# gaspachoo/EEG2Video

Measured on AMD Instinct MI355X. Metric: 6-frame 288x512 clips/sec (50-step DDIM), higher is better.
Workload: dtype f32; 1 GPU; 1xMI355X: batch=8/GPU synthetic latents [B,4,6,36,64] + [B,77,768] cond, 50-step DDIM, CFG 12.5, 288x512x6 VAE decode, fp32 (BASELINE configs[1]); clips_per_gpu=8, ddim_steps=50, unet_samples_per_ddim_step=16, weights=random-init SD-v1-4 architecture, counter RNG seed 42/43, collective=none

## Files before the change

### eeg2video_amd/_lib.py

```python
from __future__ import annotations

import ctypes as C
import os

_HERE = os.path.dirname(os.path.abspath(__file__))
LIB_PATH = os.environ.get("E2V_LIB_PATH") or os.path.join(_HERE, "lib", "libeeg2video_hip.so")

c_int64_p = C.POINTER(C.c_int64)
c_float_p = C.c_void_p


class E2VConfig(C.Structure):
    _fields_ = [
        ("in_channels", C.c_int), ("out_channels", C.c_int),
        ("block_out_channels", C.c_int * 4),
        ("layers_per_block", C.c_int), ("cross_attention_dim", C.c_int), ("attention_heads", C.c_int),
        ("norm_num_groups", C.c_int), ("norm_eps", C.c_float), ("flip_sin_to_cos", C.c_int), ("freq_shift", C.c_float),
        ("vae_in_channels", C.c_int), ("vae_latent_channels", C.c_int),
        ("vae_block_out_channels", C.c_int * 4),
        ("vae_layers_per_block", C.c_int), ("vae_norm_num_groups", C.c_int), ("vae_norm_eps", C.c_float),
        ("vae_scaling_factor", C.c_double),
        ("num_train_timesteps", C.c_int), ("beta_start", C.c_double), ("beta_end", C.c_double),
        ("steps_offset", C.c_int),
        ("sem_in_features", C.c_int), ("sem_hidden", C.c_int), ("sem_tokens", C.c_int),
# ... 27 lines not shown
    "e2v_unet_forward_ft": (_i, [_ctx, _p, C.POINTER(C.c_float), _i, _p, _i, _i, _i, _i, _i, _p, _stream]),
    "e2v_ddim_cfg_step": (_i, [_ctx, _p, _p, _p, _p, _i64, _f, _i64, _i64, _stream]),
    "e2v_vae_decode": (_i, [_ctx, _p, _i, _i, _i, _i, _i, _p, _stream]),
    "e2v_vae_encode": (_i, [_ctx, _p, _i, _i, _i, _p, _p, _stream]),
    "e2v_generate": (_i, [_ctx, _p, _p, _p, _i, _i, _i, _i, _i, _i, _i, _f, _f, _p, _p, _stream]),
    "e2v_semantic_predict": (_i, [_ctx, _p, _i, _p, _stream]),
    "e2v_dana_noise": (_i, [_ctx, _p, _p, _p, c_int64_p, _i, _f, _i, _i, _i, _i, _i, _p, _stream]),
    "e2v_frames_to_uint8": (_i, [_ctx, _p, _p, _i64, _stream]),
    "e2v_cfg_combine": (_i, [_ctx, _p, _p, _f, _p, _i64, _stream]),
    "e2v_lincomb": (_i, [_ctx, _i, C.POINTER(C.c_void_p), C.POINTER(C.c_float), _p, _i64, _stream]),
    "e2v_ddim_next_step": (_i, [_ctx, _p, _p, _p, _i64, _i64, _i, _stream]),
    "e2v_ddim_invert": (_i, [_ctx, _p, _p, _i, _i, _i, _i, _i, _i, _p, _p, _stream]),
    "e2v_set_compute_dtype": (_i, [_ctx, _i]),
    "e2v_set_conv_algo": (_i, [_ctx, _i]),
    "e2v_device_bytes": (_i64, [_ctx]),
    "e2v_comm_unique_id": (_i, [_p]),
    "e2v_comm_init": (_i, [_ctx, _p, _i, _i]),
    "e2v_comm_world": (_i, [_ctx]),
    "e2v_allgather_frames": (_i, [_ctx, _p, _i64, _i, _p, _stream]),
    "e2v_comm_destroy": (_i, [_ctx]),
    "e2v_profile_begin": (_i, [_ctx]),
    "e2v_profile_end": (_i64, [_ctx, C.c_char_p, _i64]),
    "e2v_op_conv3x3": (_i, [_ctx, _p, _i, _p, _i, _i, _i, _i, _i, _i, _i, _i, _i, _i, _p, _p, _i, _p, _i, _p, _p, _stream]),
    "e2v_op_linear": (_i, [_ctx, _p, _i, _i64, _i, _p, _p, _i, _p, _i, _p, _stream]),
    "e2v_op_groupnorm": (_i, [_ctx, _p, _i, _p, _i, _i, _i, _i, _f, _p, _p, _i, _p, _stream]),
    "e2v_op_layernorm": (_i, [_ctx, _p, _i64, _i, _p, _p, _f, _p, _stream]),
    "e2v_op_attention": (_i, [_ctx, _p, _i, _p, _p, _i, _p, _i, _i, _i, _i, _i, _i, _i, _i, _f, _stream]),
    "e2v_op_temporal_attention": (_i, [_ctx, _p, _p, _i, _i, _i, _i, _i, _f, _stream]),
    "e2v_op_to_channels_last": (_i, [_ctx, _p, _p, _i, _i, _i, _i, _stream]),
    "e2v_op_from_channels_last": (_i, [_ctx, _p, _i, _p, _i, _i, _i, _stream]),
    "e2v_op_set_knob": (_i, [C.c_char_p, _i]),
    "e2v_op_rowblock_sums": (_i, [_ctx, _p, _i64, _i, _p, _stream]),
    "e2v_op_describe_dispatch": (_i, [_ctx, _i, _i, _i, _i, _i, _i, C.c_char_p, _i64, c_int64_p]),
    "e2v_op_unet_forward_taps": (_i, [_ctx, _p, c_int64_p, _i, _p, _i, _i, _i, _i, _i, _p, _p, _i64, c_int64_p, C.POINTER(_i), _stream]),
}

_lib = None


def load() -> C.CDLL:
    global _lib
    if _lib is not None:
        return _lib
    if not os.path.isfile(LIB_PATH):
        raise ImportError(
            f"{LIB_PATH} not found: the HIP extension has not been built. "
# ... 16 lines not shown
```

### eeg2video_amd/csrc/api.cpp

```cpp
#include <cmath>
#include <cstdlib>
#include <cstring>
#include <unordered_map>
#include <mutex>

#include "../../include/eeg2video_hip_ops.h"
#include "h16.h"
#include "model.h"
#include "prof.h"

using namespace e2v;

namespace {

std::string g_create_error;

template <typename Fn>
e2v_status guarded(e2v_ctx* ctx, Fn&& fn) {
    try {
        if (ctx && !dry_run()) {
            E2V_REQUIRE(ctx->device >= 0, E2V_ESTATE, "host-only context (device = -1): no GPU work possible");
            E2V_HIP(hipSetDevice(ctx->device));
        }
        fn();
// ... 645 lines not shown
            }
        } else if (const int wm = c->conv_wino_tile(cin, cout, stride, pad_lo, Hi, Wi, Ho, Wo)) {
            Act u(c->pool, (int64_t)(wm + 2) * (wm + 2) * cout, cin);
            wino_pack_weights(w_oihw, u.p, cout, cin, wm, s);
            Act u3;
            if (c->x3_compute) {
                const size_t n = (size_t)(wm + 2) * (wm + 2) * cout * cin;
                u3 = Act(c->pool, (int64_t)((3 * n + 1) / 2 + 1023) / 1024, 1024);
                split_bf16x3(u.p, u3.p, n, n, s);
            }
            conv3_wino(c, d, wm, u.p, u3.p, nullptr, 0, s);
        } else {
            const int ld32 = conv3x3_packed_ld(cin, 32);
            Act wp(c->pool, cout, ld32);
            pack_conv3x3(w_oihw, wp.p, cout, cin, 32, s);
            IgemmArgs g = conv3_igemm(d);
            g.w = wp.p; g.ldw = ld32;
            igemm(g, s);
        }
        E2V_HIP(hipGetLastError());
    });
}

e2v_status e2v_op_linear(e2v_ctx* c, const float* x, int ldx, int64_t M, int K, const float* w, const float* bias, int N,
                         const float* resid, int geglu, float* out, e2v_stream stream) {
    if (!c) return E2V_EINVAL;
    return guarded(c, [&] {
        E2V_REQUIRE(x && w && out && (c->bf16_compute || (K % 4 == 0 && ldx % 4 == 0)), E2V_EINVAL, "bad linear arguments");
        hipStream_t s = S(c, stream);
        IgemmArgs g;
        g.a0 = x; g.c0 = K; g.lda0 = ldx; g.ldw = K; g.out = out; g.M = (int)M; g.taps = 1; g.resid = resid;
        Act wp, bp;
        if (geglu) {
            E2V_REQUIRE(N % 32 == 0 && bias, E2V_EINVAL, "GEGLU width must be a multiple of 32 and have a bias");
            wp = Act(c->pool, 2 * N, K);
            bp = Act(c->pool, 1, 2 * N);
            geglu_interleave(w, bias, N, K, wp.p, bp.p, s);
            g.w = wp.p; g.bias = bp.p; g.N = 2 * N; g.ldc = N; g.geglu = 1;
        } else {
            g.w = w; g.bias = bias; g.N = N; g.ldc = N; g.ldr = N;
        }
        Act w16, wpad, a16;
        if (c->bf16_compute) {
            const int K8 = (K + 7) / 8 * 8;
            a16 = Act(c->pool, M, K8, true);
            cvt_rows(x, ldx, 0, a16.p, K8, c->h16_mode, M, K, K8, s);
// ... 149 lines not shown
```

### eeg2video_amd/csrc/wino.hip

```cpp
#include "kernels.h"
#include "prof.h"

#include <string>

namespace e2v {

typedef float f32x4 __attribute__((ext_vector_type(4)));

__device__ __forceinline__ float wino_silu(float v) {
    return v * __builtin_amdgcn_rcpf(1.0f + __builtin_amdgcn_exp2f(v * -1.44269504088896340736f));
}

__global__ __launch_bounds__(256) void wino_in_kernel(const WinoArgs p, int img_lo, int nimg, float* __restrict__ V) {
    const int Ctot = p.c0 + p.c1;
    const int CQ = Ctot / 4;
    const int th = (p.Ho + 1) / 2, tw = (p.Wo + 1) / 2;
    const size_t T = (size_t)nimg * th * tw;
    const size_t total = T * CQ;
    const size_t plane = T * Ctot;
    for (size_t i = blockIdx.x * (size_t)blockDim.x + threadIdx.x; i < total; i += (size_t)gridDim.x * blockDim.x) {
        const size_t t = i / CQ;
        const int c = (int)(i - t * CQ) * 4;
        const int img = (int)(t / (th * tw));
        const int rem = (int)(t - (size_t)img * th * tw);
        const int ty = rem / tw, tx = rem - ty * tw;
        const bool second = c >= p.c0;
        const float* __restrict__ src = second ? p.x1 + (c - p.c0) : p.x0 + c;
        const int ld = second ? p.ld1 : p.ld0;
        const size_t img_row = (size_t)(img_lo + img) * p.Hs * p.Ws;
        f32x4 ga = {1.f, 0.f, 1.f, 0.f}, gb = {1.f, 0.f, 1.f, 0.f};
        if (p.gn_scsh) {
            const size_t slab = img_row / (size_t)p.gn_P;
            const float* sc = p.gn_scsh + (slab * Ctot + c) * 2;
            ga = *reinterpret_cast<const f32x4*>(sc);
            gb = *reinterpret_cast<const f32x4*>(sc + 4);
        }
        f32x4 d[4][4];
#pragma unroll
        for (int r = 0; r < 4; ++r) {
            const int iy = 2 * ty - 1 + r;
            const bool yok = (unsigned)iy < (unsigned)p.Ho;
            int sy = yok ? iy : 0;
            if (p.upsample) sy = min((int)floorf((float)sy * p.ups_h), p.Hs - 1);
#pragma unroll
            for (int q = 0; q < 4; ++q) {
                const int ix = 2 * tx - 1 + q;
                const bool ok = yok && (unsigned)ix < (unsigned)p.Wo;
                int sx = ok ? ix : 0;
                if (p.upsample) sx = min((int)floorf((float)sx * p.ups_w), p.Ws - 1);
                f32x4 v = {0.f, 0.f, 0.f, 0.f};
                if (ok) {
                    v = *reinterpret_cast<const f32x4*>(src + (img_row + (size_t)sy * p.Ws + sx) * ld);
                    if (p.gn_scsh) {
                        v[0] = v[0] * ga[0] + ga[1];
                        v[1] = v[1] * ga[2] + ga[3];
                        v[2] = v[2] * gb[0] + gb[1];
                        v[3] = v[3] * gb[2] + gb[3];
                        if (p.gn_silu) {
#pragma unroll
                            for (int e = 0; e < 4; ++e) v[e] = wino_silu(v[e]);
                        }
                    }
                }
                d[r][q] = v;
            }
        }
        f32x4 u[4][4];
#pragma unroll
        for (int q = 0; q < 4; ++q) {
            u[0][q] = d[0][q] - d[2][q];
            u[1][q] = d[1][q] + d[2][q];
            u[2][q] = d[2][q] - d[1][q];
            u[3][q] = d[1][q] - d[3][q];
        }
        float* __restrict__ o = V + t * Ctot + c;
#pragma unroll
        for (int r = 0; r < 4; ++r) {
            *reinterpret_cast<f32x4*>(o + (size_t)(4 * r + 0) * plane) = u[r][0] - u[r][2];
            *reinterpret_cast<f32x4*>(o + (size_t)(4 * r + 1) * plane) = u[r][1] + u[r][2];
            *reinterpret_cast<f32x4*>(o + (size_t)(4 * r + 2) * plane) = u[r][2] - u[r][1];
            *reinterpret_cast<f32x4*>(o + (size_t)(4 * r + 3) * plane) = u[r][1] - u[r][3];
        }
    }
}

__global__ __launch_bounds__(256) void wino_out_kernel(const WinoArgs p, int img_lo, int nimg, const float* __restrict__ Mb) {
    const int NQ = p.N / 4;
    const int th = (p.Ho + 1) / 2, tw = (p.Wo + 1) / 2;
    const size_t T = (size_t)nimg * th * tw;
    const size_t total = T * NQ;
    const size_t plane = T * p.N;
    for (size_t i = blockIdx.x * (size_t)blockDim.x + threadIdx.x; i < total; i += (size_t)gridDim.x * blockDim.x) {
        const size_t t = i / NQ;
        const int n = (int)(i - t * NQ) * 4;
        const int img = (int)(t / (th * tw));
        const int rem = (int)(t - (size_t)img * th * tw);
        const int ty = rem / tw, tx = rem - ty * tw;
        const float* __restrict__ m = Mb + t * p.N + n;
        f32x4 w[2][4];
#pragma unroll
        for (int q = 0; q < 4; ++q) {
            const f32x4 m0 = *reinterpret_cast<const f32x4*>(m + (size_t)(0 + q) * plane);
            const f32x4 m1 = *reinterpret_cast<const f32x4*>(m + (size_t)(4 + q) * plane);
            const f32x4 m2 = *reinterpret_cast<const f32x4*>(m + (size_t)(8 + q) * plane);
            const f32x4 m3 = *reinterpret_cast<const f32x4*>(m + (size_t)(12 + q) * plane);
            w[0][q] = m0 + m1 + m2;
            w[1][q] = m1 - m2 - m3;
        }
        f32x4 bias = {0.f, 0.f, 0.f, 0.f};
        if (p.bias) bias = *reinterpret_cast<const f32x4*>(p.bias + n);
#pragma unroll
        for (int a = 0; a < 2; ++a) {
            const int oy = 2 * ty + a;
            if (oy >= p.Ho) continue;
#pragma unroll
            for (int b = 0; b < 2; ++b) {
                const int ox = 2 * tx + b;
                if (ox >= p.Wo) continue;
                f32x4 y = b == 0 ? w[a][0] + w[a][1] + w[a][2] : w[a][1] - w[a][2] - w[a][3];
                const size_t row = ((size_t)(img_lo + img) * p.Ho + oy) * p.Wo + ox;
                y += bias;
                if (p.rowbias) y += *reinterpret_cast<const f32x4*>(p.rowbias + (row / p.rows_per_sample) * p.rb_ld + n);
                if (p.resid) y += *reinterpret_cast<const f32x4*>(p.resid + row * p.ldr + n);
                *reinterpret_cast<f32x4*>(p.out + row * p.ldc + n) = y;
            }
        }
    }
}

__device__ __forceinline__ void bt6(const f32x4 (&d)[6], f32x4 (&o)[6]) {
    o[0] = 4.f * d[0] - 5.f * d[2] + d[4];
    o[1] = -4.f * (d[1] + d[2]) + d[3] + d[4];
    o[2] = 4.f * (d[1] - d[2]) - d[3] + d[4];
    o[3] = 2.f * (d[3] - d[1]) - d[2] + d[4];
    o[4] = 2.f * (d[1] - d[3]) - d[2] + d[4];
    o[5] = 4.f * d[1] - 5.f * d[3] + d[5];
}
__device__ __forceinline__ void at6(const f32x4 (&m)[6], f32x4 (&o)[4]) {
    const f32x4 a = m[1] + m[2], b = m[1] - m[2], c = m[3] + m[4], e = m[3] - m[4];
    o[0] = m[0] + a + c;
    o[1] = b + 2.f * e;
    o[2] = a + 4.f * c;
    o[3] = b + 8.f * e + m[5];
}

__global__ __launch_bounds__(256) void wino4_in_kernel(const WinoArgs p, int img_lo, int nimg, float* __restrict__ V) {
    const int Ctot = p.c0 + p.c1;
    const int CQ = Ctot / 4;
    const int th = (p.Ho + 3) / 4, tw = (p.Wo + 3) / 4;
    const size_t T = (size_t)nimg * th * tw;
    const size_t total = T * CQ;
    const size_t plane = T * Ctot;
    for (size_t i = blockIdx.x * (size_t)blockDim.x + threadIdx.x; i < total; i += (size_t)gridDim.x * blockDim.x) {
        const size_t t = i / CQ;
        const int c = (int)(i - t * CQ) * 4;
        const int img = (int)(t / (th * tw));
        const int rem = (int)(t - (size_t)img * th * tw);
        const int ty = rem / tw, tx = rem - ty * tw;
        const bool second = c >= p.c0;
        const float* __restrict__ src = second ? p.x1 + (c - p.c0) : p.x0 + c;
        const int ld = second ? p.ld1 : p.ld0;
        const size_t img_row = (size_t)(img_lo + img) * p.Hs * p.Ws;
        f32x4 ga = {1.f, 0.f, 1.f, 0.f}, gb = {1.f, 0.f, 1.f, 0.f};
        if (p.gn_scsh) {
            const size_t slab = img_row / (size_t)p.gn_P;
            const float* sc = p.gn_scsh + (slab * Ctot + c) * 2;
            ga = *reinterpret_cast<const f32x4*>(sc);
            gb = *reinterpret_cast<const f32x4*>(sc + 4);
        }
        f32x4 u[6][6];
#pragma unroll
        for (int q = 0; q < 6; ++q) {
            const int ix = 4 * tx - 1 + q;
            const bool xok = (unsigned)ix < (unsigned)p.Wo;
            int sx = xok ? ix : 0;
            if (p.upsample) sx = min((int)floorf((float)sx * p.ups_w), p.Ws - 1);
            f32x4 d[6];
#pragma unroll
            for (int r = 0; r < 6; ++r) {
                const int iy = 4 * ty - 1 + r;
                const bool ok = xok && (unsigned)iy < (unsigned)p.Ho;
                int sy = ok ? iy : 0;
                if (p.upsample) sy = min((int)floorf((float)sy * p.ups_h), p.Hs - 1);
                f32x4 v = {0.f, 0.f, 0.f, 0.f};
                if (ok) {
                    v = *reinterpret_cast<const f32x4*>(src + (img_row + (size_t)sy * p.Ws + sx) * ld);
                    if (p.gn_scsh) {
                        v[0] = v[0] * ga[0] + ga[1];
                        v[1] = v[1] * ga[2] + ga[3];
                        v[2] = v[2] * gb[0] + gb[1];
                        v[3] = v[3] * gb[2] + gb[3];
                        if (p.gn_silu) {
#pragma unroll
                            for (int e = 0; e < 4; ++e) v[e] = wino_silu(v[e]);
                        }
                    }
                }
                d[r] = v;
            }
            f32x4 o[6];
            bt6(d, o);
#pragma unroll
            for (int r = 0; r < 6; ++r) u[r][q] = o[r];
        }
        float* __restrict__ o = V + t * Ctot + c;
#pragma unroll
        for (int r = 0; r < 6; ++r) {
            f32x4 v[6];
            bt6(u[r], v);
#pragma unroll
            for (int q = 0; q < 6; ++q) *reinterpret_cast<f32x4*>(o + (size_t)(6 * r + q) * plane) = v[q];
        }
    }
}

__global__ __launch_bounds__(256) void wino4_out_kernel(const WinoArgs p, int img_lo, int nimg, const float* __restrict__ Mb) {
    const int NQ = p.N / 4;
    const int th = (p.Ho + 3) / 4, tw = (p.Wo + 3) / 4;
    const size_t T = (size_t)nimg * th * tw;
    const size_t total = T * NQ;
    const size_t plane = T * p.N;
    for (size_t i = blockIdx.x * (size_t)blockDim.x + threadIdx.x; i < total; i += (size_t)gridDim.x * blockDim.x) {
        const size_t t = i / NQ;
        const int n = (int)(i - t * NQ) * 4;
        const int img = (int)(t / (th * tw));
        const int rem = (int)(t - (size_t)img * th * tw);
        const int ty = rem / tw, tx = rem - ty * tw;
        const float* __restrict__ m = Mb + t * p.N + n;
        f32x4 w[4][6];
#pragma unroll
        for (int q = 0; q < 6; ++q) {
            f32x4 col[6];
#pragma unroll
            for (int r = 0; r < 6; ++r) col[r] = *reinterpret_cast<const f32x4*>(m + (size_t)(6 * r + q) * plane);
            f32x4 o[4];
            at6(col, o);
#pragma unroll
            for (int a = 0; a < 4; ++a) w[a][q] = o[a];
        }
        f32x4 bias = {0.f, 0.f, 0.f, 0.f};
        if (p.bias) bias = *reinterpret_cast<const f32x4*>(p.bias + n);
#pragma unroll
        for (int a = 0; a < 4; ++a) {
            const int oy = 4 * ty + a;
            if (oy >= p.Ho) continue;
            f32x4 y[4];
            at6(w[a], y);
#pragma unroll
            for (int b = 0; b < 4; ++b) {
                const int ox = 4 * tx + b;
                if (ox >= p.Wo) continue;
                const size_t row = ((size_t)(img_lo + img) * p.Ho + oy) * p.Wo + ox;
                f32x4 v = y[b] + bias;
                if (p.rowbias) v += *reinterpret_cast<const f32x4*>(p.rowbias + (row / p.rows_per_sample) * p.rb_ld + n);
                if (p.resid) v += *reinterpret_cast<const f32x4*>(p.resid + row * p.ldr + n);
                *reinterpret_cast<f32x4*>(p.out + row * p.ldc + n) = v;
            }
        }
    }
}

__global__ void wino4_weight_kernel(const float* __restrict__ w, float* __restrict__ U, int cout, int cin) {
    const size_t total = (size_t)cout * cin;
    const float G[6][3] = {{0.25f, 0.f, 0.f}, {-1.f / 6, -1.f / 6, -1.f / 6}, {-1.f / 6, 1.f / 6, -1.f / 6},
                           {1.f / 24, 1.f / 12, 1.f / 6}, {1.f / 24, -1.f / 12, 1.f / 6}, {0.f, 0.f, 1.f}};
    for (size_t i = blockIdx.x * (size_t)blockDim.x + threadIdx.x; i < total; i += (size_t)gridDim.x * blockDim.x) {
        const float* g = w + i * 9;
        float t[6][3];
#pragma unroll
        for (int r = 0; r < 6; ++r)
#pragma unroll
            for (int x = 0; x < 3; ++x) t[r][x] = G[r][0] * g[x] + G[r][1] * g[3 + x] + G[r][2] * g[6 + x];
#pragma unroll
        for (int r = 0; r < 6; ++r)
#pragma unroll
            for (int q = 0; q < 6; ++q)
                U[(size_t)(6 * r + q) * total + i] = t[r][0] * G[q][0] + t[r][1] * G[q][1] + t[r][2] * G[q][2];
    }
}

__global__ void wino_weight_kernel(const float* __restrict__ w, float* __restrict__ U, int cout, int cin) {
// ... 20 lines not shown

void wino_pack_weights(const float* w_oihw, float* U, int cout, int cin, int m, hipStream_t s) {
    const size_t total = (size_t)cout * cin;
    const int blocks = (int)((total + 255) / 256 < 4096 ? (total + 255) / 256 : 4096);
    if (m == 4) E2V_KLAUNCH(wino4_weight_kernel, dim3(blocks), dim3(256), 0, s, w_oihw, U, cout, cin);
    else E2V_KLAUNCH(wino_weight_kernel, dim3(blocks), dim3(256), 0, s, w_oihw, U, cout, cin);
}

static inline size_t wino_tiles(const WinoArgs& a, int nimg) {
    return (size_t)nimg * ((a.Ho + a.m - 1) / a.m) * ((a.Wo + a.m - 1) / a.m);
}

size_t wino_workspace_floats(const WinoArgs& a, int nimg) {
    return (size_t)(a.m + 2) * (a.m + 2) * wino_tiles(a, nimg) * (size_t)(a.c0 + a.c1 + a.N);
}

int wino_chunk_images(const WinoArgs& a, size_t max_floats) {
    const size_t per_img = wino_workspace_floats(a, 1);
    size_t n = max_floats / (per_img ? per_img : 1);
    if (n < 1) n = 1;
    return (int)(n < (size_t)a.nimg ? n : (size_t)a.nimg);
}

void wino_conv3x3(const WinoArgs& a, float* ws, int chunk_images, hipStream_t s) {
    const int Ctot = a.c0 + a.c1;
    const int P = (a.m + 2) * (a.m + 2);
    for (int lo = 0; lo < a.nimg; lo += chunk_images) {
        const int n = a.nimg - lo < chunk_images ? a.nimg - lo : chunk_images;
        const size_t T = wino_tiles(a, n);
        float* V = ws;
        float* Mb = ws + (size_t)P * T * Ctot;
        {
            const size_t total = T * (Ctot / 4);
            const double px = (double)a.m * a.m;
            std::string nm = a.gn_scsh ? "wino_in_gn_silu" : "wino_in";
            if (prof_detail())
                nm += " T" + std::to_string(T) + " C" + std::to_string(Ctot) + " m" + std::to_string(a.m) + (a.c1 ? " cat" : "") + (a.upsample ? " up" : "");
            ProfScope ps(nm.c_str(), 2.0 * P * T * Ctot, 4.0 * ((px + P) * T * Ctot), s);
            const int blocks = (int)((total + 255) / 256 < 65536 ? (total + 255) / 256 : 65536);
            if (a.m == 4) E2V_KLAUNCH(wino4_in_kernel, dim3(blocks), dim3(256), 0, s, a, lo, n, V);
            else E2V_KLAUNCH(wino_in_kernel, dim3(blocks), dim3(256), 0, s, a, lo, n, V);
        }
        IgemmArgs g;
        g.a0 = V; g.c0 = Ctot; g.lda0 = Ctot; g.w = a.U; g.ldw = Ctot; g.ldw16 = Ctot;
        g.out = Mb; g.ldc = a.N; g.M = (int)T; g.N = a.N; g.taps = 1;
        g.batch = P; g.sa0 = (long long)T * Ctot; g.sw = (long long)a.N * Ctot; g.sout = (long long)T * a.N;
        if (a.U3) { g.x3 = 1; g.w3 = a.U3; g.w3_plane = (long long)P * a.N * Ctot; }
        igemm(g, s);
        {
            const size_t total = T * (a.N / 4);
            const double px = (double)a.m * a.m;
            std::string nm = "wino_out";
            if (prof_detail())
                nm += " T" + std::to_string(T) + " N" + std::to_string(a.N) + " m" + std::to_string(a.m) + (a.resid ? " res" : "") + (a.rowbias ? " temb" : "");
            ProfScope ps(nm.c_str(), 1.5 * P * T * a.N, 4.0 * (P * T * a.N + px * T * a.N * (a.resid ? 2 : 1)), s);
            const int blocks = (int)((total + 255) / 256 < 65536 ? (total + 255) / 256 : 65536);
            if (a.m == 4) E2V_KLAUNCH(wino4_out_kernel, dim3(blocks), dim3(256), 0, s, a, lo, n, Mb);
            else E2V_KLAUNCH(wino_out_kernel, dim3(blocks), dim3(256), 0, s, a, lo, n, Mb);
        }
    }
}

}
```

### eeg2video_amd/engine.py

```python
from __future__ import annotations

import ctypes as C
from typing import Dict, Iterable, Mapping, Optional, Sequence, Tuple

import numpy as np
import torch

from . import _lib
from .weights import SemanticConfig, UNetConfig, VAEConfig

_ERRORS = {
    _lib.E2V_EINVAL: ValueError,
    _lib.E2V_ESHAPE: ValueError,
    _lib.E2V_ENOWEIGHT: RuntimeError,
    _lib.E2V_EHIP: RuntimeError,
    _lib.E2V_ESTATE: RuntimeError,
}


def _stream() -> int:
    return torch.cuda.current_stream().cuda_stream


class Engine:
# ... 336 lines not shown

    def allgather_frames(self, frames: torch.Tensor, as_uint8: bool = False) -> torch.Tensor:
        world = self.lib.e2v_comm_world(self.ctx)
        if world <= 0:
            raise RuntimeError("allgather_frames: no communicator (Engine.comm_init first)")
        v = self._dev(frames, "frames")
        out = torch.empty((world * v.shape[0],) + tuple(v.shape[1:]), device=self.device, dtype=torch.uint8 if as_uint8 else torch.float32)
        self._check(self.lib.e2v_allgather_frames(self.ctx, v.data_ptr(), v.numel(), int(as_uint8), out.data_ptr(), _stream()))
        return out

    def op_conv3x3(self, x0, w, bias=None, x1=None, *, n_img, Hs, Ws, Hi=None, Wi=None, stride=1, pad_lo=1, pad_hi=1,
                   rowbias=None, rows_per_sample=1, resid=None):
        Hi, Wi = Hi or Hs, Wi or Ws
        Ho = (Hi + pad_lo + pad_hi - 3) // stride + 1
        Wo = (Wi + pad_lo + pad_hi - 3) // stride + 1
        cout = w.shape[0]
        out = torch.empty((n_img * Ho * Wo, cout), device=self.device, dtype=torch.float32)
        p = lambda t: t.data_ptr() if t is not None else None
        self._check(self.lib.e2v_op_conv3x3(self.ctx, x0.data_ptr(), x0.shape[1], p(x1), x1.shape[1] if x1 is not None else 0,
                                            n_img, Hs, Ws, Hi, Wi, Ho, Wo, stride, pad_lo, w.data_ptr(), p(bias), cout,
                                            p(rowbias), rows_per_sample, p(resid), out.data_ptr(), _stream()))
        return out

    def op_linear(self, x, w, bias=None, resid=None, geglu=False):
        m, k = x.shape
        n = w.shape[0] // 2 if geglu else w.shape[0]
        out = torch.empty((m, n), device=self.device, dtype=torch.float32)
        p = lambda t: t.data_ptr() if t is not None else None
        self._check(self.lib.e2v_op_linear(self.ctx, x.data_ptr(), x.stride(0), m, k, w.data_ptr(), p(bias), n, p(resid),
                                           int(geglu), out.data_ptr(), _stream()))
        return out

    def op_rowblock_sums(self, x):
        rows, c = x.shape
        out = torch.empty((rows // 64, c, 2), device=self.device, dtype=torch.float32)
        self._check(self.lib.e2v_op_rowblock_sums(self.ctx, x.data_ptr(), rows, c, out.data_ptr(), _stream()))
        return out

    def op_groupnorm(self, x0, gamma, beta, *, samples, P, groups, eps, silu=False, x1=None):
        c = x0.shape[1] + (x1.shape[1] if x1 is not None else 0)
        out = torch.empty((samples * P, c), device=self.device, dtype=torch.float32)
        self._check(self.lib.e2v_op_groupnorm(self.ctx, x0.data_ptr(), x0.shape[1], x1.data_ptr() if x1 is not None else None,
                                              x1.shape[1] if x1 is not None else 0, samples, P, groups, float(eps),
                                              gamma.data_ptr(), beta.data_ptr(), int(silu), out.data_ptr(), _stream()))
        return out

# ... 55 lines not shown
```

### include/eeg2video_hip_ops.h

```cpp
#ifndef EEG2VIDEO_HIP_OPS_H
#define EEG2VIDEO_HIP_OPS_H

#include "eeg2video_hip.h"

#ifdef __cplusplus
extern "C" {
#endif

e2v_status e2v_op_conv3x3(e2v_ctx* ctx, const float* x0, int c0, const float* x1, int c1, int n_img, int Hs, int Ws,
                          int Hi, int Wi, int Ho, int Wo, int stride, int pad_lo, const float* w_oihw, const float* bias,
                          int cout, const float* rowbias, int rows_per_sample, const float* resid, float* out,
                          e2v_stream stream);

e2v_status e2v_op_linear(e2v_ctx* ctx, const float* x, int ldx, int64_t M, int K, const float* w, const float* bias,
                         int N, const float* resid, int geglu, float* out, e2v_stream stream);

e2v_status e2v_op_groupnorm(e2v_ctx* ctx, const float* x0, int c0, const float* x1, int c1, int samples, int P,
                            int groups, float eps, const float* gamma, const float* beta, int silu, float* out,
                            e2v_stream stream);

e2v_status e2v_op_layernorm(e2v_ctx* ctx, const float* x, int64_t rows, int C, const float* gamma, const float* beta,
                            float eps, float* out, e2v_stream stream);

e2v_status e2v_op_attention(e2v_ctx* ctx, const float* q, int ldq, const float* k, const float* v, int ldkv, float* o,
                            int ldo, int n, int F, int heads, int D, int Nq, int Nk, int mode, float scale,
                            e2v_stream stream);

e2v_status e2v_op_temporal_attention(e2v_ctx* ctx, const float* qkv, float* out, int n, int F, int HW, int heads, int D,
                                     float scale, e2v_stream stream);

e2v_status e2v_op_to_channels_last(e2v_ctx* ctx, const float* in, float* out, int n, int C, int Cpad, int FHW,
                                   e2v_stream stream);
e2v_status e2v_op_from_channels_last(e2v_ctx* ctx, const float* in, int ld, float* out, int n, int C, int FHW,
                                     e2v_stream stream);

// ... 15 lines not shown
```

Measured before the change: 0.5895 clips/s.

## Specialize Winograd transform kernels by template and use 32-bit plane offsets

The Winograd input and output transform kernels become templates on GroupNorm fusion, rowbias form and residual presence, so those runtime branches drop out. All global loads are issued ahead of the arithmetic (with scheduling barriers), addresses use 32-bit per-plane offsets with a fast 32-bit divide, and out-of-range taps are masked rather than skipped. A new op entry point fuses GroupNorm+SiLU into the Winograd conv for testing. The change adds register pressure and asserts that offsets fit in 32 bits.

```diff
diff --git a/eeg2video_amd/_lib.py b/eeg2video_amd/_lib.py
--- a/eeg2video_amd/_lib.py
+++ b/eeg2video_amd/_lib.py
@@ -73,6 +73,7 @@
     "e2v_profile_begin": (_i, [_ctx]),
     "e2v_profile_end": (_i64, [_ctx, C.c_char_p, _i64]),
     "e2v_op_conv3x3": (_i, [_ctx, _p, _i, _p, _i, _i, _i, _i, _i, _i, _i, _i, _i, _i, _p, _p, _i, _p, _i, _p, _p, _stream]),
+    "e2v_op_conv3x3_gn": (_i, [_ctx, _p, _i, _p, _i, _i, _i, _i, _i, _i, _i, _i, _i, _i, _i, _i, _f, _p, _p, _p, _p, _i, _p, _i, _p, _p, _stream]),
     "e2v_op_linear": (_i, [_ctx, _p, _i, _i64, _i, _p, _p, _i, _p, _i, _p, _stream]),
     "e2v_op_groupnorm": (_i, [_ctx, _p, _i, _p, _i, _i, _i, _i, _f, _p, _p, _i, _p, _stream]),
     "e2v_op_layernorm": (_i, [_ctx, _p, _i64, _i, _p, _p, _f, _p, _stream]),
diff --git a/eeg2video_amd/csrc/api.cpp b/eeg2video_amd/csrc/api.cpp
--- a/eeg2video_amd/csrc/api.cpp
+++ b/eeg2video_amd/csrc/api.cpp
@@ -691,6 +691,51 @@
     });
 }
 
+e2v_status e2v_op_conv3x3_gn(e2v_ctx* c, const float* x0, int c0, const float* x1, int c1, int n_img, int Hs, int Ws, int Hi, int Wi,
+                             int Ho, int Wo, int stride, int pad_lo, int gn_P, int groups, float eps, const float* gamma,
+                             const float* beta, const float* w_oihw, const float* bias, int cout, const float* rowbias,
+                             int rows_per_sample, const float* resid, float* out, e2v_stream stream) {
+    if (!c) return E2V_EINVAL;
+    const int cin = c0 + c1;
+    const int64_t rows = (int64_t)n_img * Hs * Ws;
+    if (!(x0 && gamma && beta && w_oihw && out && c0 > 0 && c0 % 4 == 0 && c1 >= 0 && c1 % 4 == 0 && (c1 == 0 || x1) && cout > 0 && n_img > 0 &&
+          Hs > 0 && Ws > 0 && groups > 0 && cin % groups == 0 && gn_P > 0 && rows % gn_P == 0)) {
+        c->err = "bad conv3x3_gn arguments";
+        return E2V_EINVAL;
+    }
+    const int wm = c->conv_wino_tile(cin, cout, stride, pad_lo, Hi, Wi, Ho, Wo);
+    if (wm == 0) {
+        c->err = "conv: fused GroupNorm needs the Winograd path";
+        return E2V_ESHAPE;
+    }
+    return guarded(c, [&] {
+        hipStream_t s = S(c, stream);
+        const int samples = (int)(rows / gn_P);
+        Act part(c->pool, (int64_t)samples * groupnorm_chunks(gn_P), cin * 2);
+        Act sc(c->pool, samples, cin * 2);
+        GroupNormArgs a;
+        a.x0 = x0; a.x1 = x1; a.c0 = c0; a.c1 = c1; a.ld0 = c0; a.ld1 = c1; a.gamma = gamma; a.beta = beta;
+        a.samples = samples; a.P = gn_P; a.groups = groups; a.eps = eps;
+        a.ws_part = part.p; a.ws_scale = sc.p;
+        groupnorm_stats(a, s);
+        Conv3 d;
+        d.x0 = x0; d.c0 = c0; d.x1 = x1; d.c1 = c1; d.nimg = n_img; d.Hs = Hs; d.Ws = Ws;
+        d.Hi = Hi; d.Wi = Wi; d.Ho = Ho; d.Wo = Wo; d.stride = stride; d.pad = pad_lo;
+        d.cout = cout; d.out = out; d.bias = bias;
+        d.rowbias = rowbias; d.rb_ld = cout; d.rows_per_sample = rows_per_sample > 0 ? rows_per_sample : 1; d.resid = resid;
+        Act u(c->pool, (int64_t)(wm + 2) * (wm + 2) * cout, cin);
+        wino_pack_weights(w_oihw, u.p, cout, cin, wm, s);
+        Act u3;
+        if (c->x3_compute) {
+            const size_t n = (size_t)(wm + 2) * (wm + 2) * cout * cin;
+            u3 = Act(c->pool, (int64_t)((3 * n + 1) / 2 + 1023) / 1024, 1024);
+            split_bf16x3(u.p, u3.p, n, n, s);
+        }
+        conv3_wino(c, d, wm, u.p, u3.p, sc.p, gn_P, s);
+        E2V_HIP(hipGetLastError());
+    });
+}
+
 e2v_status e2v_op_linear(e2v_ctx* c, const float* x, int ldx, int64_t M, int K, const float* w, const float* bias, int N,
                          const float* resid, int geglu, float* out, e2v_stream stream) {
     if (!c) return E2V_EINVAL;
diff --git a/eeg2video_amd/csrc/wino.hip b/eeg2video_amd/csrc/wino.hip
--- a/eeg2video_amd/csrc/wino.hip
+++ b/eeg2video_amd/csrc/wino.hip
@@ -1,16 +1,61 @@
 #include "kernels.h"
 #include "prof.h"
-
+#include "runtime.h"
+
+#include <algorithm>
 #include <string>
 
 namespace e2v {
 
 typedef float f32x4 __attribute__((ext_vector_type(4)));
+typedef unsigned u32x4 __attribute__((ext_vector_type(4)));
 
 __device__ __forceinline__ float wino_silu(float v) {
     return v * __builtin_amdgcn_rcpf(1.0f + __builtin_amdgcn_exp2f(v * -1.44269504088896340736f));
 }
 
+__device__ __forceinline__ size_t wino_div(size_t a, size_t b) {
+    return ((a | b) >> 32) == 0 ? (size_t)((unsigned)a / (unsigned)b) : a / b;
+}
+
+#define WINO_GLOBAL __attribute__((address_space(1)))
+__device__ __forceinline__ f32x4 wino_plane_load(const float* plane_base, unsigned byte_off) {
+    asm("" : "+s"(plane_base));
+    return *reinterpret_cast<const WINO_GLOBAL f32x4*>((const WINO_GLOBAL char*)plane_base + byte_off);
+}
+__device__ __forceinline__ void wino_plane_store(float* plane_base, unsigned byte_off, f32x4 v) {
+    asm("" : "+s"(plane_base));
+    *reinterpret_cast<WINO_GLOBAL f32x4*>((WINO_GLOBAL char*)plane_base + byte_off) = v;
+}
+
+template <bool GN>
+__device__ __forceinline__ f32x4 wino_act(f32x4 v, const f32x4& ga, const f32x4& gb, bool ok) {
+    if (GN) {
+        v[0] = v[0] * ga[0] + ga[1];
+        v[1] = v[1] * ga[2] + ga[3];
+        v[2] = v[2] * gb[0] + gb[1];
+        v[3] = v[3] * gb[2] + gb[3];
+#pragma unroll
+        for (int e = 0; e < 4; ++e) v[e] = wino_silu(v[e]);
+    }
+    const u32x4 keep = ok ? ~0u : 0u;
+    return __builtin_bit_cast(f32x4, __builtin_bit_cast(u32x4, v) & keep);
+}
+
+template <int PATCH>
+__device__ __forceinline__ void wino_patch_offsets(int o0, int n_out, int n_src, bool upsample, float ups, unsigned step,
+                                                   unsigned (&off)[PATCH], bool (&ok)[PATCH]) {
+#pragma unroll
+    for (int r = 0; r < PATCH; ++r) {
+        const int i = o0 - 1 + r;
+        ok[r] = (unsigned)i < (unsigned)n_out;
+        int s = ok[r] ? i : 0;
+        if (upsample) s = min((int)floorf((float)s * ups), n_src - 1);
+        off[r] = (unsigned)s * step;
+    }
+}
+
+template <bool GN>
 __global__ __launch_bounds__(256) void wino_in_kernel(const WinoArgs p, int img_lo, int nimg, float* __restrict__ V) {
     const int Ctot = p.c0 + p.c1;
     const int CQ = Ctot / 4;
@@ -19,52 +64,36 @@
     const size_t total = T * CQ;
     const size_t plane = T * Ctot;
     for (size_t i = blockIdx.x * (size_t)blockDim.x + threadIdx.x; i < total; i += (size_t)gridDim.x * blockDim.x) {
-        const size_t t = i / CQ;
+        const size_t t = wino_div(i, CQ);
         const int c = (int)(i - t * CQ) * 4;
-        const int img = (int)(t / (th * tw));
+        const int img = (int)wino_div(t, th * tw);
         const int rem = (int)(t - (size_t)img * th * tw);
         const int ty = rem / tw, tx = rem - ty * tw;
         const bool second = c >= p.c0;
-        const float* __restrict__ src = second ? p.x1 + (c - p.c0) : p.x0 + c;
         const int ld = second ? p.ld1 : p.ld0;
         const size_t img_row = (size_t)(img_lo + img) * p.Hs * p.Ws;
+        const float* __restrict__ src = (second ? p.x1 + (c - p.c0) : p.x0 + c) + img_row * ld;
         f32x4 ga = {1.f, 0.f, 1.f, 0.f}, gb = {1.f, 0.f, 1.f, 0.f};
-        if (p.gn_scsh) {
-            const size_t slab = img_row / (size_t)p.gn_P;
+        if (GN) {
+            const size_t slab = wino_div(img_row, (size_t)p.gn_P);
             const float* sc = p.gn_scsh + (slab * Ctot + c) * 2;
             ga = *reinterpret_cast<const f32x4*>(sc);
             gb = *reinterpret_cast<const f32x4*>(sc + 4);
         }
+        unsigned yo[4], xo[4];
+        bool yok[4], xok[4];
+        wino_patch_offsets<4>(2 * ty, p.Ho, p.Hs, p.upsample, p.ups_h, (unsigned)p.Ws * ld, yo, yok);
+        wino_patch_offsets<4>(2 * tx, p.Wo, p.Ws, p.upsample, p.ups_w, (unsigned)ld, xo, xok);
         f32x4 d[4][4];
 #pragma unroll
-        for (int r = 0; r < 4; ++r) {
-            const int iy = 2 * ty - 1 + r;
-            const bool yok = (unsigned)iy < (unsigned)p.Ho;
-            int sy = yok ? iy : 0;
-            if (p.upsample) sy = min((int)floorf((float)sy * p.ups_h), p.Hs - 1);
-#pragma unroll
-            for (int q = 0; q < 4; ++q) {
-                const int ix = 2 * tx - 1 + q;
-                const bool ok = yok && (unsigned)ix < (unsigned)p.Wo;
-                int sx = ok ? ix : 0;
-                if (p.upsample) sx = min((int)floorf((float)sx * p.ups_w), p.Ws - 1);
-                f32x4 v = {0.f, 0.f, 0.f, 0.f};
-                if (ok) {
-                    v = *reinterpret_cast<const f32x4*>(src + (img_row + (size_t)sy * p.Ws + sx) * ld);
-                    if (p.gn_scsh) {
-                        v[0] = v[0] * ga[0] + ga[1];
-                        v[1] = v[1] * ga[2] + ga[3];
-                        v[2] = v[2] * gb[0] + gb[1];
-                        v[3] = v[3] * gb[2] + gb[3];
-                        if (p.gn_silu) {
-#pragma unroll
-                            for (int e = 0; e < 4; ++e) v[e] = wino_silu(v[e]);
-                        }
-                    }
-                }
-                d[r][q] = v;
-            }
-        }
+        for (int r = 0; r < 4; ++r)
+#pragma unroll
+            for (int q = 0; q < 4; ++q) d[r][q] = *reinterpret_cast<const f32x4*>(src + (yo[r] + xo[q]));
+        __builtin_amdgcn_sched_barrier(0);
+#pragma unroll
+        for (int r = 0; r < 4; ++r)
+#pragma unroll
+            for (int q = 0; q < 4; ++q) d[r][q] = wino_act<GN>(d[r][q], ga, gb, yok[r] && xok[q]);
         f32x4 u[4][4];
 #pragma unroll
         for (int q = 0; q < 4; ++q) {
@@ -73,17 +102,77 @@
             u[2][q] = d[2][q] - d[1][q];
             u[3][q] = d[1][q] - d[3][q];
         }
-        float* __restrict__ o = V + t * Ctot + c;
+        const unsigned vo = ((unsigned)t * Ctot + c) * 4u;
 #pragma unroll
         for (int r = 0; r < 4; ++r) {
-            *reinterpret_cast<f32x4*>(o + (size_t)(4 * r + 0) * plane) = u[r][0] - u[r][2];
-            *reinterpret_cast<f32x4*>(o + (size_t)(4 * r + 1) * plane) = u[r][1] + u[r][2];
-            *reinterpret_cast<f32x4*>(o + (size_t)(4 * r + 2) * plane) = u[r][2] - u[r][1];
-            *reinterpret_cast<f32x4*>(o + (size_t)(4 * r + 3) * plane) = u[r][1] - u[r][3];
-        }
-    }
-}
-
+            wino_plane_store(V + (size_t)(4 * r + 0) * plane, vo, u[r][0] - u[r][2]);
+            wino_plane_store(V + (size_t)(4 * r + 1) * plane, vo, u[r][1] + u[r][2]);
+            wino_plane_store(V + (size_t)(4 * r + 2) * plane, vo, u[r][2] - u[r][1]);
+            wino_plane_store(V + (size_t)(4 * r + 3) * plane, vo, u[r][1] - u[r][3]);
+        }
+    }
+}
+
+template <int M, int RB, bool RES>
+struct WinoTileOut {
+    float* out;
+    const float* res;
+    size_t row0;
+    unsigned yc[M], xc[M], yr[M], xr[M];
+    bool yok[M], xok[M];
+    f32x4 bias, rb;
+    f32x4 r[M][M];
+
+    __device__ __forceinline__ WinoTileOut(const WinoArgs& p, int img, int ty, int tx, int n) {
+        const int oy0 = M * ty, ox0 = M * tx;
+        row0 = ((size_t)img * p.Ho + oy0) * p.Wo + ox0;
+        out = p.out + row0 * p.ldc + n;
+        res = RES ? p.resid + row0 * p.ldr + n : nullptr;
+#pragma unroll
+        for (int a = 0; a < M; ++a) {
+            yok[a] = oy0 + a < p.Ho;
+            xok[a] = ox0 + a < p.Wo;
+            yc[a] = (unsigned)(a * p.Wo) * p.ldc;
+            xc[a] = (unsigned)a * p.ldc;
+            yr[a] = yok[a] ? (unsigned)(a * p.Wo) * p.ldr : 0u;
+            xr[a] = xok[a] ? (unsigned)a * p.ldr : 0u;
+        }
+        bias = f32x4{0.f, 0.f, 0.f, 0.f};
+        rb = bias;
+        if (p.bias) bias = *reinterpret_cast<const f32x4*>(p.bias + n);
+        if (RB == 1) rb = *reinterpret_cast<const f32x4*>(p.rowbias + wino_div(row0, (size_t)p.rows_per_sample) * p.rb_ld + n);
+    }
+    __device__ __forceinline__ void load_resid() {
+        if (!RES) return;
+#pragma unroll
+        for (int a = 0; a < M; ++a)
+#pragma unroll
+            for (int b = 0; b < M; ++b) r[a][b] = *reinterpret_cast<const f32x4*>(res + (yr[a] + xr[b]));
+    }
+    __device__ __forceinline__ void finish(const WinoArgs& p, int n, f32x4 (&y)[M][M]) const {
+#pragma unroll
+        for (int a = 0; a < M; ++a)
+#pragma unroll
+            for (int b = 0; b < M; ++b) asm volatile("" : "+v"(y[a][b]));
+        __builtin_amdgcn_s_waitcnt(0x0F70);
+#pragma unroll
+        for (int a = 0; a < M; ++a)
+#pragma unroll
+            for (int b = 0; b < M; ++b) {
+                if (!(yok[a] && xok[b])) continue;
+                f32x4 v = y[a][b] + bias;
+                if (RB == 1) v += rb;
+                if (RB == 2) {
+                    const size_t row = row0 + (size_t)a * p.Wo + b;
+                    v += *reinterpret_cast<const f32x4*>(p.rowbias + wino_div(row, (size_t)p.rows_per_sample) * p.rb_ld + n);
+                }
+                if (RES) v += r[a][b];
+                *reinterpret_cast<f32x4*>(out + (yc[a] + xc[b])) = v;
+            }
+    }
+};
+
+template <int RB, bool RES>
 __global__ __launch_bounds__(256) void wino_out_kernel(const WinoArgs p, int img_lo, int nimg, const float* __restrict__ Mb) {
     const int NQ = p.N / 4;
     const int th = (p.Ho + 1) / 2, tw = (p.Wo + 1) / 2;
@@ -91,40 +180,31 @@
     const size_t total = T * NQ;
     const size_t plane = T * p.N;
     for (size_t i = blockIdx.x * (size_t)blockDim.x + threadIdx.x; i < total; i += (size_t)gridDim.x * blockDim.x) {
-        const size_t t = i / NQ;
+        const size_t t = wino_div(i, NQ);
         const int n = (int)(i - t * NQ) * 4;
-        const int img = (int)(t / (th * tw));
+        const int img = (int)wino_div(t, th * tw);
         const int rem = (int)(t - (size_t)img * th * tw);
         const int ty = rem / tw, tx = rem - ty * tw;
-        const float* __restrict__ m = Mb + t * p.N + n;
+        const unsigned mo = ((unsigned)t * p.N + n) * 4u;
+        f32x4 mm[16];
+#pragma unroll
+        for (int k = 0; k < 16; ++k) mm[k] = wino_plane_load(Mb + (size_t)k * plane, mo);
+        WinoTileOut<2, RB, RES> tile(p, img_lo + img, ty, tx, n);
+        tile.load_resid();
+        __builtin_amdgcn_sched_barrier(0);
         f32x4 w[2][4];
 #pragma unroll
         for (int q = 0; q < 4; ++q) {
-            const f32x4 m0 = *reinterpret_cast<const f32x4*>(m + (size_t)(0 + q) * plane);
-            const f32x4 m1 = *reinterpret_cast<const f32x4*>(m + (size_t)(4 + q) * plane);
-            const f32x4 m2 = *reinterpret_cast<const f32x4*>(m + (size_t)(8 + q) * plane);
-            const f32x4 m3 = *reinterpret_cast<const f32x4*>(m + (size_t)(12 + q) * plane);
-            w[0][q] = m0 + m1 + m2;
-            w[1][q] = m1 - m2 - m3;
-        }
-        f32x4 bias = {0.f, 0.f, 0.f, 0.f};
-        if (p.bias) bias = *reinterpret_cast<const f32x4*>(p.bias + n);
+            w[0][q] = mm[q] + mm[4 + q] + mm[8 + q];
+            w[1][q] = mm[4 + q] - mm[8 + q] - mm[12 + q];
+        }
+        f32x4 y[2][2];
 #pragma unroll
         for (int a = 0; a < 2; ++a) {
-            const int oy = 2 * ty + a;
-            if (oy >= p.Ho) continue;
-#pragma unroll
-            for (int b = 0; b < 2; ++b) {
-                const int ox = 2 * tx + b;
-                if (ox >= p.Wo) continue;
-                f32x4 y = b == 0 ? w[a][0] + w[a][1] + w[a][2] : w[a][1] - w[a][2] - w[a][3];
-                const size_t row = ((size_t)(img_lo + img) * p.Ho + oy) * p.Wo + ox;
-                y += bias;
-                if (p.rowbias) y += *reinterpret_cast<const f32x4*>(p.rowbias + (row / p.rows_per_sample) * p.rb_ld + n);
-                if (p.resid) y += *reinterpret_cast<const f32x4*>(p.resid + row * p.ldr + n);
-                *reinterpret_cast<f32x4*>(p.out + row * p.ldc + n) = y;
-            }
-        }
+            y[a][0] = w[a][0] + w[a][1] + w[a][2];
+            y[a][1] = w[a][1] - w[a][2] - w[a][3];
+        }
+        tile.finish(p, n, y);
     }
 }
 
@@ -144,6 +224,7 @@
     o[3] = b + 8.f * e + m[5];
 }
 
+template <bool GN>
 __global__ __launch_bounds__(256) void wino4_in_kernel(const WinoArgs p, int img_lo, int nimg, float* __restrict__ V) {
     const int Ctot = p.c0 + p.c1;
     const int CQ = Ctot / 4;
@@ -152,68 +233,54 @@
     const size_t total = T * CQ;
     const size_t plane = T * Ctot;
     for (size_t i = blockIdx.x * (size_t)blockDim.x + threadIdx.x; i < total; i += (size_t)gridDim.x * blockDim.x) {
-        const size_t t = i / CQ;
+        const size_t t = wino_div(i, CQ);
         const int c = (int)(i - t * CQ) * 4;
-        const int img = (int)(t / (th * tw));
+        const int img = (int)wino_div(t, th * tw);
         const int rem = (int)(t - (size_t)img * th * tw);
         const int ty = rem / tw, tx = rem - ty * tw;
         const bool second = c >= p.c0;
-        const float* __restrict__ src = second ? p.x1 + (c - p.c0) : p.x0 + c;
         const int ld = second ? p.ld1 : p.ld0;
         const size_t img_row = (size_t)(img_lo + img) * p.Hs * p.Ws;
+        const float* __restrict__ src = (second ? p.x1 + (c - p.c0) : p.x0 + c) + img_row * ld;
         f32x4 ga = {1.f, 0.f, 1.f, 0.f}, gb = {1.f, 0.f, 1.f, 0.f};
-        if (p.gn_scsh) {
-            const size_t slab = img_row / (size_t)p.gn_P;
+        if (GN) {
+            const size_t slab = wino_div(img_row, (size_t)p.gn_P);
             const float* sc = p.gn_scsh + (slab * Ctot + c) * 2;
             ga = *reinterpret_cast<const f32x4*>(sc);
             gb = *reinterpret_cast<const f32x4*>(sc + 4);
         }
+        unsigned yo[6], xo[6];
+        bool yok[6], xok[6];
+        wino_patch_offsets<6>(4 * ty, p.Ho, p.Hs, p.upsample, p.ups_h, (unsigned)p.Ws * ld, yo, yok);
+        wino_patch_offsets<6>(4 * tx, p.Wo, p.Ws, p.upsample, p.ups_w, (unsigned)ld, xo, xok);
+        f32x4 d[6][6];
+#pragma unroll
+        for (int q = 0; q < 6; ++q)
+#pragma unroll
+            for (int r = 0; r < 6; ++r) d[q][r] = *reinterpret_cast<const f32x4*>(src + (yo[r] + xo[q]));
+        __builtin_amdgcn_sched_barrier(0);
         f32x4 u[6][6];
 #pragma unroll
         for (int q = 0; q < 6; ++q) {
-            const int ix = 4 * tx - 1 + q;
-            const bool xok = (unsigned)ix < (unsigned)p.Wo;
-            int sx = xok ? ix : 0;
-            if (p.upsample) sx = min((int)floorf((float)sx * p.ups_w), p.Ws - 1);
-            f32x4 d[6];
-#pragma unroll
-            for (int r = 0; r < 6; ++r) {
-                const int iy = 4 * ty - 1 + r;
-                const bool ok = xok && (unsigned)iy < (unsigned)p.Ho;
-                int sy = ok ? iy : 0;
-                if (p.upsample) sy = min((int)floorf((float)sy * p.ups_h), p.Hs - 1);
-                f32x4 v = {0.f, 0.f, 0.f, 0.f};
-                if (ok) {
-                    v = *reinterpret_cast<const f32x4*>(src + (img_row + (size_t)sy * p.Ws + sx) * ld);
-                    if (p.gn_scsh) {
-                        v[0] = v[0] * ga[0] + ga[1];
-                        v[1] = v[1] * ga[2] + ga[3];
-                        v[2] = v[2] * gb[0] + gb[1];
-                        v[3] = v[3] * gb[2] + gb[3];
-                        if (p.gn_silu) {
-#pragma unroll
-                            for (int e = 0; e < 4; ++e) v[e] = wino_silu(v[e]);
-                        }
-                    }
-                }
-                d[r] = v;
-            }
+#pragma unroll
+            for (int r = 0; r < 6; ++r) d[q][r] = wino_act<GN>(d[q][r], ga, gb, xok[q] && yok[r]);
             f32x4 o[6];
-            bt6(d, o);
+            bt6(d[q], o);
 #pragma unroll
             for (int r = 0; r < 6; ++r) u[r][q] = o[r];
         }
-        float* __restrict__ o = V + t * Ctot + c;
+        const unsigned vo = ((unsigned)t * Ctot + c) * 4u;
 #pragma unroll
         for (int r = 0; r < 6; ++r) {
             f32x4 v[6];
             bt6(u[r], v);
 #pragma unroll
-            for (int q = 0; q < 6; ++q) *reinterpret_cast<f32x4*>(o + (size_t)(6 * r + q) * plane) = v[q];
-        }
-    }
-}
-
+            for (int q = 0; q < 6; ++q) wino_plane_store(V + (size_t)(6 * r + q) * plane, vo, v[q]);
+        }
+    }
+}
+
+template <int RB, bool RES>
 __global__ __launch_bounds__(256) void wino4_out_kernel(const WinoArgs p, int img_lo, int nimg, const float* __restrict__ Mb) {
     const int NQ = p.N / 4;
     const int th = (p.Ho + 3) / 4, tw = (p.Wo + 3) / 4;
@@ -221,42 +288,32 @@
     const size_t total = T * NQ;
     const size_t plane = T * p.N;
     for (size_t i = blockIdx.x * (size_t)blockDim.x + threadIdx.x; i < total; i += (size_t)gridDim.x * blockDim.x) {
-        const size_t t = i / NQ;
+        const size_t t = wino_div(i, NQ);
         const int n = (int)(i - t * NQ) * 4;
-        const int img = (int)(t / (th * tw));
+        const int img = (int)wino_div(t, th * tw);
         const int rem = (int)(t - (size_t)img * th * tw);
         const int ty = rem / tw, tx = rem - ty * tw;
-        const float* __restrict__ m = Mb + t * p.N + n;
+        const unsigned mo = ((unsigned)t * p.N + n) * 4u;
+        f32x4 col[6][6];
+#pragma unroll
+        for (int q = 0; q < 6; ++q)
+#pragma unroll
+            for (int r = 0; r < 6; ++r) col[q][r] = wino_plane_load(Mb + (size_t)(6 * r + q) * plane, mo);
+        WinoTileOut<4, RB, RES> tile(p, img_lo + img, ty, tx, n);
+        tile.load_resid();
+        __builtin_amdgcn_sched_barrier(0);
         f32x4 w[4][6];
 #pragma unroll
         for (int q = 0; q < 6; ++q) {
-            f32x4 col[6];
-#pragma unroll
-            for (int r = 0; r < 6; ++r) col[r] = *reinterpret_cast<const f32x4*>(m + (size_t)(6 * r + q) * plane);
             f32x4 o[4];
-            at6(col, o);
+            at6(col[q], o);
 #pragma unroll
             for (int a = 0; a < 4; ++a) w[a][q] = o[a];
         }
-        f32x4 bias = {0.f, 0.f, 0.f, 0.f};
-        if (p.bias) bias = *reinterpret_cast<const f32x4*>(p.bias + n);
-#pragma unroll
-        for (int a = 0; a < 4; ++a) {
-            const int oy = 4 * ty + a;
-            if (oy >= p.Ho) continue;
-            f32x4 y[4];
-            at6(w[a], y);
-#pragma unroll
-            for (int b = 0; b < 4; ++b) {
-                const int ox = 4 * tx + b;
-                if (ox >= p.Wo) continue;
-                const size_t row = ((size_t)(img_lo + img) * p.Ho + oy) * p.Wo + ox;
-                f32x4 v = y[b] + bias;
-                if (p.rowbias) v += *reinterpret_cast<const f32x4*>(p.rowbias + (row / p.rows_per_sample) * p.rb_ld + n);
-                if (p.resid) v += *reinterpret_cast<const f32x4*>(p.resid + row * p.ldr + n);
-                *reinterpret_cast<f32x4*>(p.out + row * p.ldc + n) = v;
-            }
-        }
+        f32x4 y[4][4];
+#pragma unroll
+        for (int a = 0; a < 4; ++a) at6(w[a], y[a]);
+        tile.finish(p, n, y);
     }
 }
 
@@ -323,9 +380,26 @@
     return (int)(n < (size_t)a.nimg ? n : (size_t)a.nimg);
 }
 
+using WinoInKernel = void (*)(const WinoArgs, int, int, float*);
+using WinoOutKernel = void (*)(const WinoArgs, int, int, const float*);
+
 void wino_conv3x3(const WinoArgs& a, float* ws, int chunk_images, hipStream_t s) {
     const int Ctot = a.c0 + a.c1;
     const int P = (a.m + 2) * (a.m + 2);
+    const int ldmax = std::max(std::max(a.ld0, a.ld1), std::max(a.ldc, a.ldr));
+    E2V_REQUIRE((uint64_t)a.Hs * a.Ws * ldmax < ((uint64_t)1 << 32) && (uint64_t)(a.m + 1) * a.Wo * ldmax < ((uint64_t)1 << 32) &&
+                    (uint64_t)wino_tiles(a, std::min(chunk_images, a.nimg)) * std::max(Ctot, a.N) < ((uint64_t)1 << 30),
+                E2V_ESHAPE, "winograd conv: an image or a transform plane exceeds 32-bit offsets");
+    E2V_REQUIRE(!a.gn_scsh || a.gn_silu, E2V_EINVAL, "winograd conv: the fused GroupNorm comes with its SiLU");
+    static const WinoInKernel in_kernels[2][2] = {{wino_in_kernel<false>, wino_in_kernel<true>}, {wino4_in_kernel<false>, wino4_in_kernel<true>}};
+    static const WinoOutKernel out_kernels[2][3][2] = {
+        {{wino_out_kernel<0, false>, wino_out_kernel<0, true>}, {wino_out_kernel<1, false>, wino_out_kernel<1, true>},
+         {wino_out_kernel<2, false>, wino_out_kernel<2, true>}},
+        {{wino4_out_kernel<0, false>, wino4_out_kernel<0, true>}, {wino4_out_kernel<1, false>, wino4_out_kernel<1, true>},
+         {wino4_out_kernel<2, false>, wino4_out_kernel<2, true>}}};
+    const int rb_form = !a.rowbias ? 0 : a.rows_per_sample % (a.Ho * a.Wo) == 0 ? 1 : 2;
+    const WinoInKernel in_kernel = in_kernels[a.m == 4][a.gn_scsh != nullptr];
+    const WinoOutKernel out_kernel = out_kernels[a.m == 4][rb_form][a.resid != nullptr];
     for (int lo = 0; lo < a.nimg; lo += chunk_images) {
         const int n = a.nimg - lo < chunk_images ? a.nimg - lo : chunk_images;
         const size_t T = wino_tiles(a, n);
@@ -339,8 +413,7 @@
                 nm += " T" + std::to_string(T) + " C" + std::to_string(Ctot) + " m" + std::to_string(a.m) + (a.c1 ? " cat" : "") + (a.upsample ? " up" : "");
             ProfScope ps(nm.c_str(), 2.0 * P * T * Ctot, 4.0 * ((px + P) * T * Ctot), s);
             const int blocks = (int)((total + 255) / 256 < 65536 ? (total + 255) / 256 : 65536);
-            if (a.m == 4) E2V_KLAUNCH(wino4_in_kernel, dim3(blocks), dim3(256), 0, s, a, lo, n, V);
-            else E2V_KLAUNCH(wino_in_kernel, dim3(blocks), dim3(256), 0, s, a, lo, n, V);
+            E2V_KLAUNCH(in_kernel, dim3(blocks), dim3(256), 0, s, a, lo, n, V);
         }
         IgemmArgs g;
         g.a0 = V; g.c0 = Ctot; g.lda0 = Ctot; g.w = a.U; g.ldw = Ctot; g.ldw16 = Ctot;
@@ -356,10 +429,9 @@
                 nm += " T" + std::to_string(T) + " N" + std::to_string(a.N) + " m" + std::to_string(a.m) + (a.resid ? " res" : "") + (a.rowbias ? " temb" : "");
             ProfScope ps(nm.c_str(), 1.5 * P * T * a.N, 4.0 * (P * T * a.N + px * T * a.N * (a.resid ? 2 : 1)), s);
             const int blocks = (int)((total + 255) / 256 < 65536 ? (total + 255) / 256 : 65536);
-            if (a.m == 4) E2V_KLAUNCH(wino4_out_kernel, dim3(blocks), dim3(256), 0, s, a, lo, n, Mb);
-            else E2V_KLAUNCH(wino_out_kernel, dim3(blocks), dim3(256), 0, s, a, lo, n, Mb);
-        }
-    }
-}
-
-}
+            E2V_KLAUNCH(out_kernel, dim3(blocks), dim3(256), 0, s, a, lo, n, Mb);
+        }
+    }
+}
+
+}
diff --git a/eeg2video_amd/engine.py b/eeg2video_amd/engine.py
--- a/eeg2video_amd/engine.py
+++ b/eeg2video_amd/engine.py
@@ -382,6 +382,20 @@
                                             p(rowbias), rows_per_sample, p(resid), out.data_ptr(), _stream()))
         return out
 
+    def op_conv3x3_gn(self, x0, gamma, beta, w, bias=None, x1=None, *, n_img, Hs, Ws, gn_P, groups, eps, Hi=None, Wi=None, stride=1,
+                      pad_lo=1, pad_hi=1, rowbias=None, rows_per_sample=1, resid=None):
+        Hi, Wi = Hi or Hs, Wi or Ws
+        Ho = (Hi + pad_lo + pad_hi - 3) // stride + 1
+        Wo = (Wi + pad_lo + pad_hi - 3) // stride + 1
+        cout = w.shape[0]
+        out = torch.empty((n_img * Ho * Wo, cout), device=self.device, dtype=torch.float32)
+        p = lambda t: t.data_ptr() if t is not None else None
+        self._check(self.lib.e2v_op_conv3x3_gn(self.ctx, x0.data_ptr(), x0.shape[1], p(x1), x1.shape[1] if x1 is not None else 0,
+                                               n_img, Hs, Ws, Hi, Wi, Ho, Wo, stride, pad_lo, gn_P, groups, float(eps),
+                                               gamma.data_ptr(), beta.data_ptr(), w.data_ptr(), p(bias), cout, p(rowbias),
+                                               rows_per_sample, p(resid), out.data_ptr(), _stream()))
+        return out
+
     def op_linear(self, x, w, bias=None, resid=None, geglu=False):
         m, k = x.shape
         n = w.shape[0] // 2 if geglu else w.shape[0]
diff --git a/include/eeg2video_hip_ops.h b/include/eeg2video_hip_ops.h
--- a/include/eeg2video_hip_ops.h
+++ b/include/eeg2video_hip_ops.h
@@ -11,6 +11,11 @@
                           int Hi, int Wi, int Ho, int Wo, int stride, int pad_lo, const float* w_oihw, const float* bias,
                           int cout, const float* rowbias, int rows_per_sample, const float* resid, float* out,
                           e2v_stream stream);
+
+e2v_status e2v_op_conv3x3_gn(e2v_ctx* ctx, const float* x0, int c0, const float* x1, int c1, int n_img, int Hs, int Ws, int Hi, int Wi,
+                             int Ho, int Wo, int stride, int pad_lo, int gn_P, int groups, float eps, const float* gamma,
+                             const float* beta, const float* w_oihw, const float* bias, int cout, const float* rowbias,
+                             int rows_per_sample, const float* resid, float* out, e2v_stream stream);
 
 e2v_status e2v_op_linear(e2v_ctx* ctx, const float* x, int ldx, int64_t M, int K, const float* w, const float* bias,
                          int N, const float* resid, int geglu, float* out, e2v_stream stream);
```

After: 0.5955 clips/s, median of 6. 1.01x the previous value.
